# jacobkrantz/IVLN-CE

Hardware: AMD Instinct MI355X
Metric: env-steps/sec (batched MapCMA fwd+bwd) at 1/2/4/8 MI355X; t-nDTW parity (higher is better)
Workload: dtype f32

## Files before the change

ivln-ce_amd/build.py:

```python
import os
import subprocess
import sys

HERE = os.path.dirname(os.path.abspath(__file__))
CSRC = os.path.join(HERE, "csrc")
OUT = os.path.join(HERE, "libivln_hip.so")

SOURCES = {
    "mapper.hip": ["-ffp-contract=off"],
    "gemm_conv.hip": ["-mllvm", "-pragma-unroll-threshold=200000"],
    "conv_direct.hip": [],
    "gemm_vec.hip": ["-mllvm", "-pragma-unroll-threshold=200000"],
    "conv1x1_stream.hip": [],
    "conv_bf3.hip": [],
    "gn_conv.hip": [],
    "depth_net.hip": [],
    "cma_step.hip": [],
    "state_rnn.hip": [],
    "instr_rnn.hip": [],
    "nn_ops.hip": [],
    "train_ops.hip": [],
    "dtw.cpp": [],
}
COMMON = ["--offload-arch=gfx950", "-O3", "-std=c++17", "-fPIC", "-Wall", "-Wno-unused-function"]


def _stale(target, deps):
    if not os.path.exists(target):
        return True
    t = os.path.getmtime(target)
    return any(os.path.getmtime(d) > t for d in deps)


def build_all(force=False, verbose=True):
    hipcc = os.environ.get("HIPCC", "/opt/rocm/bin/hipcc")
    objs = []
    headers = [os.path.join(CSRC, f) for f in os.listdir(CSRC) if f.endswith((".h", ".hpp"))]
    headers.append(os.path.join(HERE, "..", "include", "ivln_hip.h"))
    procs = []
    for src, extra in SOURCES.items():
        s = os.path.join(CSRC, src)
        o = os.path.join(CSRC, src.rsplit(".", 1)[0] + ".o")
        objs.append(o)
        if force or _stale(o, [s] + headers):
            cmd = [hipcc] + COMMON + extra + ["-c", s, "-o", o]
            if verbose:
                print(" ".join(cmd), flush=True)
            procs.append((src, subprocess.Popen(cmd)))
    for src, p in procs:
        if p.wait() != 0:
            raise RuntimeError(f"hipcc failed on {src}")
    if force or procs or _stale(OUT, objs):
        cmd = [hipcc, "--offload-arch=gfx950", "-shared", "-fPIC", "-o", OUT] + objs
        if verbose:
            print(" ".join(cmd), flush=True)
        subprocess.check_call(cmd)
    return OUT


if __name__ == "__main__":
    build_all(force="--force" in sys.argv)
```

ivln-ce_amd/csrc/conv_bf3.hip:

```cpp
#include <stdlib.h>

#include <type_traits>

#include "bf3_common.h"
#include "residency.h"

namespace {

#ifdef BF3_TIMING
__device__ unsigned long long g_bf3_stamp[8192 * 8];
#endif

template <int KS, int TM, int WM, int WN, int PTH, int PTW, int IMGS, int DA, bool FUSE = false, int ST = 1>
__global__ __launch_bounds__(64 * WM * WN, 2) void k_conv_bf3(const ivln_gemm_desc p, const unsigned char* a_split, long long a_grp_bytes,
                                                           int tiles_w, int tiles_h, int nimg, int chunks_per_split) {
#ifdef BF3_TIMING
    const unsigned long long t_entry = threadIdx.x == 0 ? wall_clock64() : 0ull;
#endif
    constexpr int NTB = 64 * WM * WN, TN = 2;
    constexpr int BM = 32 * TM * WM, BN = 32 * TN * WN;
    static_assert(IMGS * PTH * PTW == BN && PTW % 4 == 0, "pixel tile");
    constexpr int KK = KS * KS, KKP = bf3_taps_padded(KS), CS = bf3_stage_chunks(KS);
    constexpr int RP = KKP * CS;
    static_assert(RP % DA == 0 && KKP >= KK && (CS == 1 || KK == 1), "prefetch rotation closes over a stage");
// ... 956 lines not shown
    float* const red = reinterpret_cast<float*>(smem);
    bf3_red_put<LDT>(red, wave, half, l31, acc);
    __syncthreads();
#pragma unroll
    for (int it = 0; it < ITEMS; ++it) {
        const int item = t + it * 512, ml = item >> 5, q = item & 31;
        float4 v = bf3_red_sum<NW, LDT, float4, 32>(red + ml * LDT + q);
        if (eoff[it] >= 0) {
            const int64_t addr = eoff[it];
            const float sc = esc[it], sh = esh[it];
            if (p.scale) v.x = fmaf(v.x, sc, sh), v.y = fmaf(v.y, sc, sh), v.z = fmaf(v.z, sc, sh), v.w = fmaf(v.w, sc, sh);
            else if (p.shift) v.x += sh, v.y += sh, v.z += sh, v.w += sh;
            const bool res_pre = p.residual && !p.residual_after_relu, res_post = p.residual && p.residual_after_relu;
            if (res_pre)
                v.x += __int_as_float(rres[it][0]), v.y += __int_as_float(rres[it][1]), v.z += __int_as_float(rres[it][2]),
                    v.w += __int_as_float(rres[it][3]);
            if (p.accumulate) {
                const float4 ra = *reinterpret_cast<const float4*>(p.D + addr);
                v.x += ra.x, v.y += ra.y, v.z += ra.z, v.w += ra.w;
            }
            if (p.relu) v.x = fmaxf(v.x, 0.f), v.y = fmaxf(v.y, 0.f), v.z = fmaxf(v.z, 0.f), v.w = fmaxf(v.w, 0.f);
            if (res_post)
                v.x += __int_as_float(rres[it][0]), v.y += __int_as_float(rres[it][1]), v.z += __int_as_float(rres[it][2]),
                    v.w += __int_as_float(rres[it][3]);
            *reinterpret_cast<float4*>(p.D + addr) = v;
        }
    }
    }
#ifdef BF3_TIMING
    if (lane == 0) {
        __builtin_amdgcn_s_waitcnt(0);
        const unsigned long long ts3 = wall_clock64();
        const int b = ((blockIdx.y * gridDim.x + blockIdx.x) * NW + wave) & 8191;
        g_bf3_stamp[b * 8 + 0] = ts1 - ts0;
        g_bf3_stamp[b * 8 + 1] = ts2 - ts1;
        g_bf3_stamp[b * 8 + 2] = ts3 - ts2;
        g_bf3_stamp[b * 8 + 3] = ts0;
        g_bf3_stamp[b * 8 + 4] = tc_split;
        g_bf3_stamp[b * 8 + 5] = tc_load;
        g_bf3_stamp[b * 8 + 6] = tc_mfma;
    }
#endif
}

int bf3_1x1_ks_launch(ivln_gemm_desc& d, hipStream_t s, int mode, int form_pin = -1) {
    if (d.stride != 1 || d.pad != 0 || d.Cin % CB != 0 || d.Cin < 4 * CB || d.stat_partials || d.splits > 1) return IVLN_E_UNSUPPORTED;
    if ((d.HoWo & 3) || (d.in_img_stride & 3) || ((((uintptr_t)d.B) | ((uintptr_t)d.D) | ((uintptr_t)d.residual)) & 15)) return IVLN_E_UNSUPPORTED;
    const int64_t nimg = d.N / d.HoWo;
    if (nimg * d.in_img_stride * 4 >= (int64_t)1 << 31 || nimg * d.Ctot * d.HoWo * 4 >= (int64_t)1 << 31) return IVLN_E_UNSUPPORTED;
    if (d.grp_imgs > 0 && ((int64_t)d.grp_imgs * d.HoWo) % 128 != 0) return IVLN_E_UNSUPPORTED;
    const int nch = d.Cin / CB;
    bool wt = nch <= 16;
    if (nch == 32 && (int64_t)((d.N + 127) / 128) * ((d.M + 31) / 32) > 2 * (int64_t)ivln_cu_count()) wt = true;
    if (form_pin >= 0) wt = form_pin == 1;
    if (wt && nch > 64) wt = false;
    if (wt && d.accumulate) return IVLN_E_UNSUPPORTED;
    const int64_t mtiles = (d.M + 31) / 32;
    const int64_t wgs = wt ? (int64_t)((d.N + 511) / 512) * mtiles : (int64_t)((d.N + 127) / 128) * mtiles;
    if ((d.N + 127) / 128 > 65535) return IVLN_E_UNSUPPORTED;
    if (mode == 0) {
        if (!wt && (d.Cin < 32 * CB || wgs > 2 * (int64_t)ivln_cu_count() || wgs < ivln_cu_count() / 2)) return IVLN_E_UNSUPPORTED;
        if (wt && wgs < ivln_cu_count()) return IVLN_E_UNSUPPORTED;
    }
    d.splits = 1;
    const unsigned char* a = (const unsigned char*)d.A_split;
    const long long gb = (long long)(d.a_split_grp_stride * 4);
    if (wt) {
        constexpr size_t lds = 0;
        dim3 grid((unsigned)mtiles, (unsigned)((d.N + 511) / 512), 1);
        IVLN_LAUNCH_FAMILY(k_conv1x1_bf3_ks<true>, grid, dim3(256), lds, s, d, a, gb);
    } else {
        constexpr size_t lds = (size_t)8 * 32 * (128 + 4) * 4;
        if (bf3_set_lds<k_conv1x1_bf3_ks<false>>(lds) != IVLN_OK) return IVLN_E_HIP;
        dim3 grid((unsigned)mtiles, (unsigned)((d.N + 127) / 128), 1);
        IVLN_LAUNCH_FAMILY(k_conv1x1_bf3_ks<false>, grid, dim3(512), lds, s, d, a, gb);
    }
    return IVLN_OK;
}

__global__ __launch_bounds__(256) void k_conv_bf3_pack(const float* __restrict__ W, int M, int Cin, int KS, uint16_t* __restrict__ out,
                                                       int64_t total) {
    const int64_t idx = (int64_t)blockIdx.x * 256 + threadIdx.x;
    if (idx >= total) return;
    const int KK = KS * KS, KKP = bf3_taps_padded(KS), nch = (Cin + CB - 1) / CB;
    const int e = (int)(idx & 7), lane = (int)((idx >> 3) & 63);
    int64_t q = idx >> 9;
    const int pl = (int)(q % 3);
    q /= 3;
    const int r = (int)(q % KKP);
    q /= KKP;
    const int c = (int)(q % nch);
    const int mt = (int)(q / nch);
    const int m = mt * 32 + (lane & 31), ci = c * CB + (lane >> 5) * 8 + e;
    const float v = (m < M && ci < Cin && r < KK) ? W[((int64_t)m * Cin + ci) * KK + r] : 0.f;
    uint32_t h, mm, l;
    split3(v, h, mm, l);
    out[idx] = (uint16_t)(pl == 0 ? h : (pl == 1 ? mm : l));
}

template <int KS, int TM, int WM, int WN, int PTH, int PTW, int IMGS, int DA, int ST = 1>
int launch_bf3(const ivln_gemm_desc& d, hipStream_t s, const unsigned char* a_split, int64_t grp_bytes, int nimg, int cps) {
    constexpr int NTB = 64 * WM * WN, BM = 32 * TM * WM, BN = 64 * WN;
    constexpr int PH = ST == 2 ? PTH + 1 : PTH + KS - 1, PWR = ST == 2 ? PTW + 1 : PTW + KS - 1;
    constexpr int NPIX = IMGS * (ST == 2 ? 4 : 1) * PH * PWR * bf3_stage_chunks(KS);
    constexpr size_t lds = (size_t)(NPIX * PIXB > 32 * (BN + 4) * 4 ? NPIX * PIXB : 32 * (BN + 4) * 4);
    if constexpr (lds > 160 * 1024) {
// ... 755 lines not shown
```

ivln-ce_amd/csrc/nn_ops.hip:

```cpp
#include <hip/hip_runtime.h>
#include <stdint.h>
#include <math.h>
#include "../../include/ivln_hip.h"

namespace {

__device__ __forceinline__ float wave_sum(float v) {
#pragma unroll
    for (int o = 32; o > 0; o >>= 1) v += __shfl_xor(v, o);
    return v;
}
__device__ __forceinline__ float wave_max(float v) {
#pragma unroll
    for (int o = 32; o > 0; o >>= 1) v = fmaxf(v, __shfl_xor(v, o));
    return v;
}
__device__ __forceinline__ float block_sum(float v, float* red) {
    v = wave_sum(v);
    int w = threadIdx.x >> 6, nw = (blockDim.x + 63) >> 6;
    __syncthreads();
    if ((threadIdx.x & 63) == 0) red[w] = v;
    __syncthreads();
    float s = 0.f;
    for (int i = 0; i < nw; ++i) s += red[i];
    return s;
}
__device__ __forceinline__ float block_max(float v, float* red) {
    v = wave_max(v);
    int w = threadIdx.x >> 6, nw = (blockDim.x + 63) >> 6;
    __syncthreads();
    if ((threadIdx.x & 63) == 0) red[w] = v;
    __syncthreads();
    float s = -INFINITY;
    for (int i = 0; i < nw; ++i) s = fmaxf(s, red[i]);
    return s;
}

constexpr int GN_CACHE = 8192;
constexpr int GN_THREADS = 512;

__device__ __forceinline__ float4 gn_load4(const float* __restrict__ xp, int i, int HW, int64_t chan_stride,
                                           int splits, int64_t slab_stride) {
    int cl = i / HW, pp = i - cl * HW;
    const float* p = xp + (int64_t)cl * chan_stride + pp;
    float4 v = *reinterpret_cast<const float4*>(p);
    int z = 1;
    for (; z + 3 < splits; z += 4) {
        float4 w0 = *reinterpret_cast<const float4*>(p + (int64_t)z * slab_stride);
        float4 w1 = *reinterpret_cast<const float4*>(p + (int64_t)(z + 1) * slab_stride);
        float4 w2 = *reinterpret_cast<const float4*>(p + (int64_t)(z + 2) * slab_stride);
        float4 w3 = *reinterpret_cast<const float4*>(p + (int64_t)(z + 3) * slab_stride);
        v.x += (w0.x + w1.x) + (w2.x + w3.x);
        v.y += (w0.y + w1.y) + (w2.y + w3.y);
        v.z += (w0.z + w1.z) + (w2.z + w3.z);
        v.w += (w0.w + w1.w) + (w2.w + w3.w);
    }
// ... 346 lines not shown
        float2 t2 = *reinterpret_cast<const float2*>(xp + (int64_t)z * slab_stride);
        float2 u2 = *reinterpret_cast<const float2*>(xp + (int64_t)z * slab_stride + W);
        t.x += t2.x; t.y += t2.y; u.x += u2.x; u.y += u2.y;
    }
    for (int off = lpo >> 1; off > 0; off >>= 1) {
        t.x += __shfl_xor(t.x, off, 64);
        t.y += __shfl_xor(t.y, off, 64);
        u.x += __shfl_xor(u.x, off, 64);
        u.y += __shfl_xor(u.y, off, 64);
    }
    if (!live || sub != 0) return;
    const float sc = scale[c], sh = shift[c];
    float a = fmaxf(fmaf(t.x, sc, sh), 0.f);
    float b = fmaxf(fmaf(t.y, sc, sh), 0.f);
    float c2 = fmaxf(fmaf(u.x, sc, sh), 0.f);
    float d = fmaxf(fmaf(u.y, sc, sh), 0.f);
    y[idx] = (((a + b) + c2) + d) * 0.25f;
}

__global__ __launch_bounds__(256) void k_pool2d(const float* __restrict__ x, float* __restrict__ y, int NC, int H,
                                                int W, int Ho, int Wo, int k, int s, int p, int mode) {
    int64_t idx = (int64_t)blockIdx.x * 256 + threadIdx.x;
    if (idx >= (int64_t)NC * Ho * Wo) return;
    int wo = (int)(idx % Wo);
    int ho = (int)((idx / Wo) % Ho);
    int nc = (int)(idx / ((int64_t)Wo * Ho));
    const float* xp = x + (int64_t)nc * H * W;
    float acc = mode == 0 ? -INFINITY : 0.f;
    for (int i = 0; i < k; ++i) {
        int h = ho * s - p + i;
        if ((unsigned)h >= (unsigned)H) continue;
        for (int j = 0; j < k; ++j) {
            int w = wo * s - p + j;
            if ((unsigned)w >= (unsigned)W) continue;
            float v = xp[(int64_t)h * W + w];
            acc = mode == 0 ? fmaxf(acc, v) : acc + v;
        }
    }
    if (mode == 1) acc = acc / (float)(k * k);
    y[idx] = acc;
}

__global__ __launch_bounds__(256) void k_subsample2_x4(const float* __restrict__ x, float* __restrict__ y, int64_t total4, int H, int W,
                                                      int Ho, int Wo) {
    const int64_t idx = (int64_t)blockIdx.x * 256 + threadIdx.x;
    if (idx >= total4) return;
    const int W4 = Wo >> 2;
    const int j = (int)(idx % W4);
    const int ho = (int)((idx / W4) % Ho);
    const int64_t nc = idx / ((int64_t)W4 * Ho);
    const float4* r = reinterpret_cast<const float4*>(x + (nc * H + 2 * ho) * W + 8 * j);
    const float4 a = r[0], b = r[1];
    *reinterpret_cast<float4*>(y + (nc * Ho + ho) * Wo + 4 * j) = make_float4(a.x, a.z, b.x, b.z);
}

__global__ __launch_bounds__(256) void k_maxpool3s2p1_x4(const float* __restrict__ x, float* __restrict__ y, int64_t total4, int H, int W,
                                                        int Ho, int Wo) {
    const int64_t idx = (int64_t)blockIdx.x * 256 + threadIdx.x;
    if (idx >= total4) return;
    const int W4 = Wo >> 2;
    const int j = (int)(idx % W4);
    const int ho = (int)((idx / W4) % Ho);
    const int64_t nc = idx / ((int64_t)W4 * Ho);
    const float* xp = x + nc * H * W;
    float m[9];
#pragma unroll
    for (int k = 0; k < 9; ++k) m[k] = -INFINITY;
#pragma unroll
    for (int i = 0; i < 3; ++i) {
        const int h = 2 * ho - 1 + i;
        if ((unsigned)h < (unsigned)H) {
            const float* r = xp + (int64_t)h * W + 8 * j;
            const float4 a = *reinterpret_cast<const float4*>(r), b = *reinterpret_cast<const float4*>(r + 4);
            const float l = j > 0 ? r[-1] : -INFINITY;
            m[0] = fmaxf(m[0], l), m[1] = fmaxf(m[1], a.x), m[2] = fmaxf(m[2], a.y), m[3] = fmaxf(m[3], a.z), m[4] = fmaxf(m[4], a.w);
            m[5] = fmaxf(m[5], b.x), m[6] = fmaxf(m[6], b.y), m[7] = fmaxf(m[7], b.z), m[8] = fmaxf(m[8], b.w);
        }
    }
    float4 o;
    o.x = fmaxf(fmaxf(m[0], m[1]), m[2]), o.y = fmaxf(fmaxf(m[2], m[3]), m[4]);
    o.z = fmaxf(fmaxf(m[4], m[5]), m[6]), o.w = fmaxf(fmaxf(m[6], m[7]), m[8]);
    *reinterpret_cast<float4*>(y + (nc * Ho + ho) * Wo + 4 * j) = o;
}

__global__ __launch_bounds__(256) void k_map_features(const uint8_t* __restrict__ occ,
                                                      const uint8_t* __restrict__ sem, float* __restrict__ y,
                                                      int B, int cells, int classes) {
    int64_t idx = (int64_t)blockIdx.x * 256 + threadIdx.x;
    int64_t total = (int64_t)B * (1 + classes) * cells;
    if (idx >= total) return;
    int p = (int)(idx % cells);
    int c = (int)((idx / cells) % (1 + classes));
    int b = (int)(idx / ((int64_t)cells * (1 + classes)));
    float v;
    if (c == 0) v = (float)occ[(int64_t)b * cells + p];
    else v = sem[(int64_t)b * cells + p] == (uint8_t)(c - 1) ? 1.f : 0.f;
    y[idx] = v;
}

__global__ __launch_bounds__(256) void k_map_features4(const uint8_t* __restrict__ occ, const uint8_t* __restrict__ sem,
                                                       float* __restrict__ y, int B, int cells, int classes) {
    const int64_t q = (int64_t)blockIdx.x * 256 + threadIdx.x;
    const int cq = cells >> 2;
    const int64_t total = (int64_t)B * (1 + classes) * cq;
    if (q >= total) return;
    const int p4 = (int)(q % cq);
// ... 881 lines not shown
                           const float* u_sample, const float* u_beta, float beta, const double* expert,
                           int64_t* action, float* logits_out, void* stream) {
    if (O > 8 || O <= 0 || (K & 3) || (ldx & 3) || rows <= 0) return IVLN_E_UNSUPPORTED;
    if (!u_sample || (u_beta && !expert)) return IVLN_E_INVALID;
    hipLaunchKernelGGL(k_linear_argmax<true>, dim3(1), dim3(256), 0, (hipStream_t)stream, x, ldx, W, bias, rows, K, O,
                       action, logits_out, u_sample, u_beta, beta, expert);
    return LAUNCH_OK();
}

int ivln_rgb_to_nchw_f32(const uint8_t* rgb, int B, int H, int W, float div, float* out, void* stream) {
    if (B <= 0 || div == 0.f) return IVLN_E_INVALID;
    hipLaunchKernelGGL(k_rgb_to_nchw, dim3(nblk((int64_t)B * H * W)), dim3(256), 0, (hipStream_t)stream, rgb, B, H, W,
                       div, out);
    return LAUNCH_OK();
}

int ivln_adaptive_avgpool2d_f32(const float* x, int N, int C, int H, int W, int OH, int OW, float* out,
                                int64_t out_img_stride, void* stream) {
    if (N <= 0 || OH <= 0 || OW <= 0) return IVLN_E_INVALID;
    if (out_img_stride <= 0) out_img_stride = (int64_t)C * OH * OW;
    hipLaunchKernelGGL(k_adaptive_avgpool2d, dim3(nblk((int64_t)N * C * OH * OW)), dim3(256), 0, (hipStream_t)stream, x,
                       N, C, H, W, OH, OW, out, out_img_stride);
    return LAUNCH_OK();
}

int ivln_argmax_channels_u8(const float* x, int N, int C, int HW, uint8_t* out, void* stream) {
    hipLaunchKernelGGL(k_argmax_channels_u8, dim3(nblk((int64_t)N * HW)), dim3(256), 0, (hipStream_t)stream, x, N, C,
                       HW, out);
    return LAUNCH_OK();
}

int ivln_rgb_resize_normalize_f32(const uint8_t* rgb, int B, int Hi, int Wi, int Ho, int Wo, float* out,
                                  void* stream) {
    if (Hi == Ho && Wi == Wo && ((int64_t)Ho * Wo) % 4 == 0 && !((uintptr_t)rgb & 3) && !((uintptr_t)out & 15)) {
        const int64_t quads = (int64_t)B * Ho * Wo / 4;
        hipLaunchKernelGGL(k_rgb_normalize_x4, dim3(nblk(quads)), dim3(256), 0, (hipStream_t)stream, rgb, quads, Ho * Wo, out);
        return LAUNCH_OK();
    }
    hipLaunchKernelGGL(k_rgb_resize_normalize, dim3(nblk((int64_t)B * 3 * Ho * Wo)), dim3(256), 0,
                       (hipStream_t)stream, rgb, B, Hi, Wi, Ho, Wo, out);
    return LAUNCH_OK();
}

int ivln_affine_f32(const float* x, float* y, int64_t n, float sub, float div, void* stream) {
    hipLaunchKernelGGL(k_affine, dim3(nblk(n)), dim3(256), 0, (hipStream_t)stream, x, y, n, sub, div);
    return LAUNCH_OK();
}

int ivln_add_f32(const float* a, const float* b, float* y, int64_t n, int relu, void* stream) {
    hipLaunchKernelGGL(k_add, dim3(nblk(n)), dim3(256), 0, (hipStream_t)stream, a, b, y, n, relu);
    return LAUNCH_OK();
}

int ivln_copy2d_f32(const float* src, int64_t ld_src, float* dst, int64_t ld_dst, int rows, int cols,
                    int broadcast_rows, void* stream) {
    hipLaunchKernelGGL(k_copy2d, dim3(nblk((int64_t)rows * cols)), dim3(256), 0, (hipStream_t)stream, src, ld_src,
                       dst, ld_dst, rows, cols, broadcast_rows);
    return LAUNCH_OK();
}

int ivln_copy_multi(const void* const* srcs, void* const* dsts, const int64_t* bytes, int n, void* stream) {
    if (n < 0 || n > 8) return IVLN_E_INVALID;
    CopyJobs J;
    int blocks = 0, m = 0;
    for (int j = 0; j < n; ++j) {
        if (bytes[j] <= 0) continue;
        if (!srcs[j] || !dsts[j]) return IVLN_E_INVALID;
        J.src[m] = (const uint8_t*)srcs[j];
        J.dst[m] = (uint8_t*)dsts[j];
        J.bytes[m] = bytes[j];
        J.first_block[m] = blocks;
        blocks += (int)((bytes[j] + COPY_CHUNK - 1) / COPY_CHUNK);
        ++m;
    }
    if (m == 0) return IVLN_OK;
    J.first_block[m] = blocks;
    J.n = m;
    hipLaunchKernelGGL(k_copy_multi, dim3(blocks), dim3(256), 0, (hipStream_t)stream, J);
    return LAUNCH_OK();
}

int ivln_rednet_fwd(const ivln_rednet_op* table, int n_ops, const uint8_t* rgb, const float* depth, uint8_t* labels_out,
                    void* stream) {
    if (!table || n_ops <= 0) return IVLN_E_INVALID;
    for (int k = 0; k < n_ops; ++k) {
        const ivln_rednet_op& op = table[k];
        int rc = IVLN_E_INVALID;
        switch (op.kind) {
            case IVLN_OP_GEMM:
                rc = ivln_gemm_f32(&op.gemm, stream);
                break;
            case IVLN_OP_ADD:
                rc = ivln_add_f32((const float*)op.src0, (const float*)op.src1, (float*)op.dst, op.n, op.i[0], stream);
                break;
            case IVLN_OP_POOL:
                rc = ivln_pool2d_f32((const float*)op.src0, (float*)op.dst, op.i[0], op.i[1], op.i[2], op.i[3], op.i[4],
                                     op.i[5], op.i[6], stream);
                break;
            case IVLN_OP_RGB_NORM: {
                const uint8_t* src = op.src0 ? (const uint8_t*)op.src0 : rgb;
                if (src)
                    rc = ivln_rgb_resize_normalize_f32(src, op.i[0], op.i[1], op.i[2], op.i[3], op.i[4], (float*)op.dst,
                                                       stream);
                break;
            }
            case IVLN_OP_AFFINE: {
                const float* src = op.src0 ? (const float*)op.src0 : depth;
                if (src) rc = ivln_affine_f32(src, (float*)op.dst, op.n, op.f[0], op.f[1], stream);
                break;
            }
            case IVLN_OP_ARGMAX_U8: {
                uint8_t* dst = op.dst ? (uint8_t*)op.dst : labels_out;
                if (dst) rc = ivln_argmax_channels_u8((const float*)op.src0, op.i[0], op.i[1], op.i[2], dst, stream);
                break;
            }
            default:
                break;
        }
        if (rc != IVLN_OK) return rc;
    }
    return IVLN_OK;
}

int ivln_add_multi_f32(const float* const* srcs, float* const* dsts, const int64_t* counts, int n, void* stream) {
    if (n < 0 || n > 64) return IVLN_E_INVALID;
    AddJobs J;
    int blocks = 0, m = 0;
    for (int j = 0; j < n; ++j) {
        if (counts[j] <= 0) continue;
        if (!srcs[j] || !dsts[j]) return IVLN_E_INVALID;
        J.src[m] = srcs[j];
        J.dst[m] = dsts[j];
        J.n[m] = counts[j];
        J.first_block[m] = blocks;
        blocks += (int)((counts[j] + ADD_CHUNK - 1) / ADD_CHUNK);
        ++m;
    }
    if (m == 0) return IVLN_OK;
    J.first_block[m] = blocks;
    J.count = m;
    hipLaunchKernelGGL(k_add_multi, dim3(blocks), dim3(256), 0, (hipStream_t)stream, J);
    return LAUNCH_OK();
}

}
```

ivln-ce_amd/ops.py:

```python
import ctypes as C
import contextlib
import functools
import os
from typing import Optional

import torch

from . import _lib
from ._lib import check, f32, i32, i64, lib, stream_ptr, vp
from ._lib import dptr as _dptr


class GemmDesc(C.Structure):

    _fields_ = [
        ("A", vp), ("B", vp), ("D", vp),
        ("M", i32), ("N", i32), ("K", i32),
        ("amode", i32), ("bmode", i32), ("dmode", i32),
        ("lda", i64), ("ldb", i64),
        ("Cin", i32), ("Hin", i32), ("Win", i32), ("Hout", i32), ("Wout", i32),
        ("stride", i32), ("pad", i32), ("dil", i32),
        ("koff", vp), ("kpos", vp),
        ("HoWo", i32), ("Ctot", i32),
        ("in_img_stride", i64),
        ("sDm", i64), ("sDn", i64),
        ("scale", vp), ("shift", vp), ("residual", vp),
        ("relu", i32), ("accumulate", i32),
        ("splits", i32),
        ("ws", vp), ("ws_floats", i64),
        ("defer_epilogue", i32), ("splits_used", C.POINTER(i32)),
        ("tile_override", i32),
        ("A_packed", vp),
        ("no_xcd_remap", i32),
        ("grp_imgs", i32), ("a_grp_stride", i64), ("a_packed_grp_stride", i64),
        ("no_wide_epilogue", i32),
        ("stat_partials", vp), ("stat_tiles", C.POINTER(i32)),
        ("A_split", vp), ("a_split_grp_stride", i64),
        ("split_ok", i32),
        ("img_run_flags", vp),
        ("fuse_A_split", vp), ("fuse_a_grp_stride", i64), ("fuse_scale", vp), ("fuse_shift", vp), ("fuse_M", i32),
        ("residual_after_relu", i32),
        ("real_taps", i32),
        ("pool2", i32), ("map_sem_u8", vp),
    ]


class RednetOp(C.Structure):
    _fields_ = [("kind", i32), ("i", i32 * 7), ("f", f32 * 2), ("n", i64), ("src0", vp), ("src1", vp), ("dst", vp),
                ("gemm", GemmDesc)]


OP_GEMM, OP_ADD, OP_POOL, OP_RGB_NORM, OP_AFFINE, OP_ARGMAX_U8 = range(6)


class OpRecorder:

    def __init__(self):
        self.ops, self.keep, self.unsupported = [], [], []

    def table(self):
        arr = (RednetOp * len(self.ops))()
        for k, op in enumerate(self.ops):
            C.memmove(C.byref(arr, k * C.sizeof(RednetOp)), C.byref(op), C.sizeof(RednetOp))
        return arr


_REC = None


class recording:
    def __enter__(self):
        global _REC
        if _REC is not None:
            raise _lib.IvlnError("ops.recording() does not nest")
        _REC = OpRecorder()
        return _REC

    def __exit__(self, *exc):
        global _REC
        _REC = None
        return False


def _rec(kind, ints=(), floats=(), n=0, src0=None, src1=None, dst=None, gemm=None):
    op = RednetOp()
    op.kind = kind
    for k, v in enumerate(ints):
        op.i[k] = int(v)
    for k, v in enumerate(floats):
        op.f[k] = float(v)
    op.n, op.src0, op.src1, op.dst = int(n), src0, src1, dst
    if gemm is not None:
        C.memmove(C.byref(op, RednetOp.gemm.offset), C.byref(gemm), C.sizeof(GemmDesc))
        op.gemm.splits_used = None
    _REC.ops.append(op)


A_MK, A_KM, A_NCHW_P = 0, 1, 2
B_CONV, B_CONV1X1, B_KN, B_NK, B_IM2COL_T, B_CONVT, B_CONV_K3, B_CONV_K7, B_CONV_K2 = 0, 1, 2, 3, 4, 5, 6, 7, 8
D_NCHW, D_DENSE, D_NCHW_UP2, D_NCHW_UP2X4 = 0, 1, 2, 3

_sigs_done = False


def _L():
    global _sigs_done
    L = lib()
    if not _sigs_done:
        L.ivln_gemm_f32.argtypes = [C.POINTER(GemmDesc), vp]
        L.ivln_groupnorm_f32.argtypes = [vp, vp, vp, vp, vp, i32, i32, i32, i32, f32, i32, i64, i64, i32, i64, i64, i64,
                                         vp, vp, vp]
        L.ivln_bn_fold_f32.argtypes = [vp, vp, vp, vp, vp, f32, i32, vp, vp, vp]
        L.ivln_bn_train_stats_f32.argtypes = [vp, i32, i32, i32, vp, vp, vp, vp, f32, f32, vp, vp, vp, vp, vp, i64, vp]
        L.ivln_scale_shift_relu_avgpool2_f32.argtypes = [vp, vp, vp, vp, i32, i32, i32, i32, i64, i64, i32, i64, vp]
        L.ivln_pool2d_f32.argtypes = [vp, vp, i32, i32, i32, i32, i32, i32, i32, vp]
        L.ivln_map_features_f32.argtypes = [vp, vp, vp, i32, i32, i32, vp]
        L.ivln_embed_lengths.argtypes = [vp, vp, i32, i32, i32, i32, vp, vp, vp]
        L.ivln_embed_gates_dirs_f32.argtypes = [vp, vp, vp, i32, i32, i32, i32, i32, vp, vp, vp, vp, vp, vp]
        L.ivln_lstm_dirs_fwd_f32.argtypes = [vp] * 7 + [i32, i32, i32, i32, vp, vp, vp, vp, i32, vp, vp]
        L.ivln_gru_dirs_fwd_f32.argtypes = [vp] * 7 + [i32, i32, i32, i32, vp, vp, vp, vp]
        L.ivln_linear_skinny_f32.argtypes = [vp, i64, vp, vp, vp, i64, i32, i32, i32, i32, vp]
        L.ivln_gru_step_f32.argtypes = [vp, i64, i32, vp, i64, vp, i64, vp, vp, vp, vp, vp, vp, i64, vp, i64, i32, i32,
                                        vp, vp, vp, vp, vp]
        L.ivln_attn_fwd_f32.argtypes = [vp, i64, vp, i64, vp, i64, vp, f32, i32, i32, i32, i32, vp, i64, vp, vp, vp]
        L.ivln_prev_action_embed_f32.argtypes = [vp, vp, vp, i32, i32, i32, vp, i64, vp, i64, vp]
        L.ivln_argmax_rows.argtypes = [vp, i32, i32, vp, vp]
        L.ivln_argmax_channels_u8.argtypes = [vp, i32, i32, i32, vp, vp]
        L.ivln_rgb_resize_normalize_f32.argtypes = [vp, i32, i32, i32, i32, i32, vp, vp]
        L.ivln_affine_f32.argtypes = [vp, vp, i64, f32, f32, vp]
        L.ivln_add_f32.argtypes = [vp, vp, vp, i64, i32, vp]
        L.ivln_copy2d_f32.argtypes = [vp, i64, vp, i64, i32, i32, i32, vp]
        L.ivln_tour_memory_f32.argtypes = [vp, i64, vp, i64, vp, i32, i32, vp, i64, vp, i64, vp]
        L.ivln_seq_sync_init.argtypes = L.ivln_seq_sync_status.argtypes = [vp, vp]
        L.ivln_cma_seq_fwd_f32.argtypes = [vp, vp, i64, vp, vp, vp, vp, i64, vp, i64, i32, i32, i32, vp, vp, vp, vp, vp, vp]
        L.ivln_lstm_step_f32.argtypes = [vp, i64, i32, vp, i64, vp, i64, vp, i64, vp, vp, vp, vp, vp, vp, i64, vp, i64, vp,
                                         i64, i32, i32, vp, vp, vp, vp, vp, vp]
        L.ivln_lstm_seq_fwd_f32.argtypes = [vp, vp, i64, vp, i64, vp, vp, vp, vp, i64, vp, i64, vp, i64, i32, i32, i32, vp,
                                            vp, vp, vp, vp, vp]
        L.ivln_lstm_seq_bwd_f32.argtypes = [vp, i64, vp, vp, vp, vp, vp, vp, i64, vp, i64, vp, i64, vp, vp, i32, i32, i32,
                                            vp, vp, vp, i64, vp, i64, vp]
        _sigs_done = True
    return L


def dptr(t: torch.Tensor) -> int:
    if _REC is not None:
        _REC.keep.append(t)
    return _dptr(t)


def _p(t: Optional[torch.Tensor]):
    if t is None:
        return None
    if not t.is_cuda:
        raise _lib.IvlnError("HIP hot path needs GPU tensors (no CPU fallback); got " + str(t.device))
    if _REC is not None:
        _REC.keep.append(t)
    return t.data_ptr()


_tables = {}
_ws = {}


def conv_tables(cin, kh, kw, hin, win, dil, device, transposed=False):
    key = (cin, kh, kw, hin, win, dil, str(device), transposed)
    t = _tables.get(key)
    if t is None:
        ci = torch.arange(cin, dtype=torch.int64).view(-1, 1, 1)
        a = torch.arange(kh, dtype=torch.int64).view(1, -1, 1)
        b = torch.arange(kw, dtype=torch.int64).view(1, 1, -1)
        if transposed:
            koff = (ci * hin * win + 0 * a + 0 * b).reshape(-1)
        else:
            koff = (ci * hin * win + a * dil * win + b * dil).reshape(-1)
        kpos = (0 * ci + (a << 16) + b).reshape(-1)
        t = (koff.to(torch.int32).to(device), kpos.to(torch.int32).to(device))
        _tables[key] = t
    return t


def splitk_ws(device, floats=8 << 20, slot=0):
    key = (str(device), stream_ptr(), slot)
# ... 1189 lines not shown
    check(_L().ivln_argmax_channels_u8(dptr(x), N, Cc, H * W, dptr(out), stream_ptr()), "ivln_argmax_channels_u8")
    if _REC is not None:
        _rec(OP_ARGMAX_U8, (N, Cc, H * W), src0=x.data_ptr(), dst=None)
    return out


def rgb_resize_normalize(rgb_u8_nhwc, Ho, Wo):
    B, Hi, Wi, _ = rgb_u8_nhwc.shape
    out = torch.empty((B, 3, Ho, Wo), dtype=torch.float32, device=rgb_u8_nhwc.device)
    check(_L().ivln_rgb_resize_normalize_f32(dptr(rgb_u8_nhwc), B, Hi, Wi, Ho, Wo, dptr(out), stream_ptr()),
          "ivln_rgb_resize_normalize_f32")
    if _REC is not None:
        _rec(OP_RGB_NORM, (B, Hi, Wi, Ho, Wo), src0=None, dst=out.data_ptr())
    return out


def rgb_to_nchw(rgb_u8_nhwc, div=255.0):
    B, H, W, _ = rgb_u8_nhwc.shape
    out = torch.empty((B, 3, H, W), dtype=torch.float32, device=rgb_u8_nhwc.device)
    L = _L()
    L.ivln_rgb_to_nchw_f32.argtypes = [vp, i32, i32, i32, f32, vp, vp]
    check(L.ivln_rgb_to_nchw_f32(dptr(rgb_u8_nhwc), B, H, W, div, dptr(out), stream_ptr()), "ivln_rgb_to_nchw_f32")
    return out


def adaptive_avgpool2d(x, OH, OW, out=None, out_ctot=0):
    N, Cc, H, W = x.shape
    if out is None:
        out = torch.empty((N, Cc, OH, OW), dtype=torch.float32, device=x.device)
    L = _L()
    L.ivln_adaptive_avgpool2d_f32.argtypes = [vp, i32, i32, i32, i32, i32, i32, vp, i64, vp]
    check(L.ivln_adaptive_avgpool2d_f32(dptr(x), N, Cc, H, W, OH, OW, _p(out), out_ctot * OH * OW, stream_ptr()),
          "ivln_adaptive_avgpool2d_f32")
    return out


def affine(x, sub, div):
    out = torch.empty_like(x)
    check(_L().ivln_affine_f32(dptr(x), dptr(out), x.numel(), sub, div, stream_ptr()), "ivln_affine_f32")
    if _REC is not None:
        _rec(OP_AFFINE, floats=(sub, div), n=x.numel(), src0=None, dst=out.data_ptr())
    return out


def add(a, b, relu=False, out=None):
    if out is None:
        out = torch.empty_like(a)
    check(_L().ivln_add_f32(dptr(a), dptr(b), dptr(out), a.numel(), int(bool(relu)), stream_ptr()), "ivln_add_f32")
    if _REC is not None:
        _rec(OP_ADD, (int(bool(relu)),), n=a.numel(), src0=a.data_ptr(), src1=b.data_ptr(), dst=out.data_ptr())
    return out


def copy_multi(pairs):
    L = _L()
    L.ivln_copy_multi.argtypes = [C.POINTER(C.c_void_p), C.POINTER(C.c_void_p), C.POINTER(C.c_int64), C.c_int,
                                  C.c_void_p]
    for k in range(0, len(pairs), 8):
        chunk = pairs[k:k + 8]
        n = len(chunk)
        srcs, dsts, nb = (C.c_void_p * n)(), (C.c_void_p * n)(), (C.c_int64 * n)()
        for i, (s, d) in enumerate(chunk):
            if s.shape != d.shape or s.dtype != d.dtype or not s.is_contiguous() or not d.is_contiguous():
                raise _lib.IvlnError("copy_multi needs contiguous tensors of identical shape and dtype")
            srcs[i], dsts[i], nb[i] = _p(s), _p(d), s.numel() * s.element_size()
        check(L.ivln_copy_multi(srcs, dsts, nb, n, stream_ptr()), "ivln_copy_multi")


def add_multi(pairs):
    L = _L()
    L.ivln_add_multi_f32.argtypes = [C.POINTER(C.c_void_p), C.POINTER(C.c_void_p), C.POINTER(C.c_int64), C.c_int,
                                     C.c_void_p]
    for k in range(0, len(pairs), 64):
        chunk = pairs[k:k + 64]
        n = len(chunk)
        srcs, dsts, cnt = (C.c_void_p * n)(), (C.c_void_p * n)(), (C.c_int64 * n)()
        for i, (s, d) in enumerate(chunk):
            if (s.numel() != d.numel() or s.dtype != torch.float32 or d.dtype != torch.float32
                    or not s.is_contiguous() or not d.is_contiguous()):
                raise _lib.IvlnError("add_multi needs contiguous float32 tensors of identical size")
            srcs[i], dsts[i], cnt[i] = _p(s), _p(d), s.numel()
        check(L.ivln_add_multi_f32(srcs, dsts, cnt, n, stream_ptr()), "ivln_add_multi_f32")


def tour_memory(mem, h, mask_u8, out1, out2=None):
    N, H = mem.shape
    check(
        _L().ivln_tour_memory_f32(_p(mem), mem.stride(0), _p(h) if h is not None else None, h.stride(0) if h is not None else 0,
                                  _p(mask_u8) if mask_u8 is not None else None, N, H, _p(out1), out1.stride(0),
                                  _p(out2) if out2 is not None else None, out2.stride(0) if out2 is not None else 0,
                                  stream_ptr()),
        "ivln_tour_memory_f32",
    )
    return out1


def copy2d(src, dst, rows, cols, broadcast_rows=False):
    check(
        _L().ivln_copy2d_f32(_p(src), src.stride(0) if src.dim() > 1 else cols, _p(dst), dst.stride(0), rows, cols,
                             int(bool(broadcast_rows)), stream_ptr()),
        "ivln_copy2d_f32",
    )


_tsigs_done = False

# ... 375 lines not shown
```

ivln-ce_amd/rednet.py:

```python
import os

import torch
import torch.nn as nn

from . import ops


GROUP_ENCODERS = True


def _conv3x3(cin, cout, stride=1):
    return nn.Conv2d(cin, cout, kernel_size=3, stride=stride, padding=1, bias=False)


class _Folded:

    def __init__(self):
        self.c = {}

    def bn(self, bn: nn.BatchNorm2d):
        k = id(bn)
        if k not in self.c:
            C = bn.num_features
            scale = torch.empty(C, dtype=torch.float32, device=bn.weight.device)
            shift = torch.empty(C, dtype=torch.float32, device=bn.weight.device)
            ops.bn_fold(bn, scale, shift)
            self.c[k] = (scale, shift)
        return self.c[k]

    def pair(self, conv_a, bn_a, conv_b, bn_b):
        k = ("pair", id(conv_a))
        if k not in self.c:
            (sa, ba), (sb, bb) = self.bn(bn_a), self.bn(bn_b)
            w = torch.stack([conv_a.weight.detach(), conv_b.weight.detach()]).contiguous()
            self.c[k] = (w, torch.cat([sa, sb]).contiguous(), torch.cat([ba, bb]).contiguous())
        return self.c[k]

    def classes(self, convt: nn.ConvTranspose2d):
        k = ("cls", id(convt))
        if k not in self.c:
            ok = convt.stride == (2, 2) and convt.kernel_size[0] == convt.kernel_size[1] and \
                2 - 2 * convt.padding[0] + convt.kernel_size[0] - 2 + convt.output_padding[0] == 2
            cls = ops.convt_s2_classes(convt.weight.detach(), convt.padding[0]) if ok else None
            self.c[k] = None if cls is None else (cls, ops.convt_s2_stack(cls))
        return self.c[k]

    def wt(self, convt: nn.ConvTranspose2d):
        k = id(convt)
        if k not in self.c:
            self.c[k] = convt.weight.detach().permute(1, 0, 2, 3).contiguous()
        return self.c[k]


def _convt(x, convt: nn.ConvTranspose2d, f: _Folded, **epi):
    cls = f.classes(convt)
    if cls is not None:
        return ops.conv_transpose2d_s2(x, cls[0], stacked=cls[1], **epi)
    return ops.conv_transpose2d(x, f.wt(convt), convt.stride[0], convt.padding[0], convt.output_padding[0], **epi)


STAGE_HOOK = None


def _stage_done(name):
    if STAGE_HOOK is not None:
        STAGE_HOOK(name)


SKIP_ADD_FUSED = os.environ.get("IVLN_REDNET_SKIP_ADD", "1") != "0"


class Bottleneck(nn.Module):
    expansion = 4

    def __init__(self, inplanes, planes, stride=1, downsample=None):
        super().__init__()
        self.conv1 = nn.Conv2d(inplanes, planes, kernel_size=1, bias=False)
        self.bn1 = nn.BatchNorm2d(planes)
        self.conv2 = nn.Conv2d(planes, planes, kernel_size=3, stride=stride, padding=1, bias=False)
        self.bn2 = nn.BatchNorm2d(planes)
        self.conv3 = nn.Conv2d(planes, planes * 4, kernel_size=1, bias=False)
        self.bn3 = nn.BatchNorm2d(planes * 4)
        self.relu = nn.ReLU(inplace=True)
        self.downsample = downsample
        self.stride = stride

    def forward_hip(self, x, f: _Folded):
        residual = x
        if self.downsample is not None:
            s, b = f.bn(self.downsample[1])
            residual = ops.conv2d(x, self.downsample[0].weight, stride=self.stride, scale=s, shift=b)
        s, b = f.bn(self.bn1)
        y = ops.conv2d(x, self.conv1.weight, scale=s, shift=b, relu=True)
        s, b = f.bn(self.bn2)
        s3, b3 = f.bn(self.bn3)
        if self.stride == 1:
            out = ops.conv3x3_then_1x1(y, self.conv2.weight, s, b, self.conv3.weight, s3, b3, residual)
            if out is not None:
                return out
        y = ops.conv2d(y, self.conv2.weight, stride=self.stride, pad=1, scale=s, shift=b, relu=True)
        return ops.conv2d(y, self.conv3.weight, scale=s3, shift=b3, residual=residual, relu=True)


def _conv_pair(x2, w2, s2, b2, stride=1, pad=0, residual=None, relu=False):
    N, _, H, W = x2.shape
    G, Cout, _, KH, KW = w2.shape
    B = N // G
    Ho, Wo = (H + 2 * pad - KH) // stride + 1, (W + 2 * pad - KW) // stride + 1
    if (B * Ho * Wo) % 32 == 0:
        return ops.conv2d(x2, w2, stride=stride, pad=pad, scale=s2, shift=b2, residual=residual, relu=relu)
    out = torch.empty((N, Cout, Ho, Wo), dtype=torch.float32, device=x2.device)
    for g in range(G):
        sl = slice(g * B, (g + 1) * B)
        ops.conv2d(x2[sl], w2[g], stride=stride, pad=pad, scale=s2[g * Cout:(g + 1) * Cout], shift=b2[g * Cout:(g + 1) * Cout],
                   residual=residual[sl] if residual is not None else None, relu=relu, out=out[sl])
    return out


def _bottleneck_pair(blk: Bottleneck, blk_d: Bottleneck, x2, f: _Folded):
    residual = x2
    if blk.downsample is not None:
        w, s, b = f.pair(blk.downsample[0], blk.downsample[1], blk_d.downsample[0], blk_d.downsample[1])
        residual = _conv_pair(x2, w, s, b, stride=blk.stride)
    w, s, b = f.pair(blk.conv1, blk.bn1, blk_d.conv1, blk_d.bn1)
    y = _conv_pair(x2, w, s, b, relu=True)
    w, s, b = f.pair(blk.conv2, blk.bn2, blk_d.conv2, blk_d.bn2)
    w3, s3, b3 = f.pair(blk.conv3, blk.bn3, blk_d.conv3, blk_d.bn3)
    if blk.stride == 1:
        out = ops.conv3x3_then_1x1(y, w, s, b, w3, s3, b3, residual)
        if out is not None:
            return out
    y = _conv_pair(y, w, s, b, stride=blk.stride, pad=1, relu=True)
    return _conv_pair(y, w3, s3, b3, residual=residual, relu=True)


class TransBasicBlock(nn.Module):
    expansion = 1

    def __init__(self, inplanes, planes, stride=1, upsample=None, **kwargs):
        super().__init__()
        self.conv1 = _conv3x3(inplanes, inplanes)
        self.bn1 = nn.BatchNorm2d(inplanes)
        self.relu = nn.ReLU(inplace=True)
        if upsample is not None and stride != 1:
            self.conv2 = nn.ConvTranspose2d(inplanes, planes, kernel_size=3, stride=stride, padding=1,
                                            output_padding=1, bias=False)
        else:
            self.conv2 = _conv3x3(inplanes, planes, stride)
        self.bn2 = nn.BatchNorm2d(planes)
        self.upsample = upsample
        self.stride = stride

    def forward_hip(self, x, f: _Folded):
        residual = x
        if self.upsample is not None:
            s, b = f.bn(self.upsample[1])
            up = self.upsample[0]
            if isinstance(up, nn.ConvTranspose2d):
                residual = _convt(x, up, f, scale=s, shift=b)
            else:
                residual = ops.conv2d(x, up.weight, scale=s, shift=b)
        s, b = f.bn(self.bn1)
        y = ops.conv2d(x, self.conv1.weight, pad=1, scale=s, shift=b, relu=True)
        s, b = f.bn(self.bn2)
        if isinstance(self.conv2, nn.ConvTranspose2d):
            return _convt(y, self.conv2, f, scale=s, shift=b, residual=residual, relu=True)
        return ops.conv2d(y, self.conv2.weight, stride=self.stride, pad=1, scale=s, shift=b, residual=residual,
                          relu=True)


class RedNet(nn.Module):
    def __init__(self, cfg):
# ... 55 lines not shown
            upsample = nn.Sequential(
                nn.ConvTranspose2d(self.inplanes, planes, kernel_size=2, stride=stride, padding=0, bias=False),
                nn.BatchNorm2d(planes),
            )
        elif self.inplanes != planes:
            upsample = nn.Sequential(
                nn.Conv2d(self.inplanes, planes, kernel_size=1, stride=stride, bias=False), nn.BatchNorm2d(planes)
            )
        layers = [block(self.inplanes, self.inplanes) for _ in range(1, blocks)]
        layers.append(block(self.inplanes, planes, stride, upsample))
        self.inplanes = planes
        return nn.Sequential(*layers)

    def _make_agant_layer(self, inplanes, planes):
        return nn.Sequential(
            nn.Conv2d(inplanes, planes, kernel_size=1, stride=1, padding=0, bias=False),
            nn.BatchNorm2d(planes), nn.ReLU(inplace=True),
        )

    def invalidate_folded(self):
        self._folded = _Folded()

    def _seq(self, seq, x):
        for blk in seq:
            x = blk.forward_hip(x, self._folded)
        return x

    def _agant(self, layer, x):
        s, b = self._folded.bn(layer[1])
        return ops.conv2d(x, layer[0].weight, scale=s, shift=b, relu=True)

    def _skip_add(self, up, layer, fuse):
        s, b = self._folded.bn(layer[1])
        out = ops.conv2d(fuse, layer[0].weight, scale=s, shift=b, residual=up, relu=True, residual_after_relu=True) if SKIP_ADD_FUSED else None
        return out if out is not None else ops.add(up, self._agant(layer, fuse))

    def forward(self, rgb, depth):
        assert not self.training, "HIP RedNet is inference-only (the reference freezes it, mapper.py:751-752)"
        f = self._folded
        if GROUP_ENCODERS:
            B = rgb.shape[0]
            S = torch.empty((2 * B, 64, rgb.shape[2] // 2, rgb.shape[3] // 2), dtype=torch.float32, device=rgb.device)
            s, b = f.bn(self.bn1)
            sd, bd = f.bn(self.bn1_d)
            ops.conv2d(depth, self.conv1_d.weight, stride=2, pad=3, scale=sd, shift=bd, relu=True, out=S[B:])
            fuse0 = ops.conv2d(rgb, self.conv1.weight, stride=2, pad=3, scale=s, shift=b, relu=True, out=S[:B], residual=S[B:],
                               residual_after_relu=True) if ops.BF3_STEM else None
            if fuse0 is None:
                ops.conv2d(rgb, self.conv1.weight, stride=2, pad=3, scale=s, shift=b, relu=True, out=S[:B])
                fuse0 = ops.add(S[:B], S[B:], out=S[:B])
            P = ops.pool2d(S, 3, 2, 1, "max")
            fuses = []
            _stage_done("stem")
            for li, (la, lb) in enumerate(((self.layer1, self.layer1_d), (self.layer2, self.layer2_d),
                                           (self.layer3, self.layer3_d), (self.layer4, self.layer4_d))):
                for blk, blk_d in zip(la, lb):
                    P = _bottleneck_pair(blk, blk_d, P, f)
                fuses.append(ops.add(P[:B], P[B:], out=P[:B]))
                _stage_done(f"layer{li + 1}")
            fuse1, fuse2, fuse3, fuse4 = fuses
        else:
            s, b = f.bn(self.bn1)
            x = ops.conv2d(rgb, self.conv1.weight, stride=2, pad=3, scale=s, shift=b, relu=True)
            s, b = f.bn(self.bn1_d)
            d = ops.conv2d(depth, self.conv1_d.weight, stride=2, pad=3, scale=s, shift=b, relu=True)
            fuse0 = ops.add(x, d)
            x = ops.pool2d(fuse0, 3, 2, 1, "max")
            d = ops.pool2d(d, 3, 2, 1, "max")
            x, d = self._seq(self.layer1, x), self._seq(self.layer1_d, d)
            fuse1 = ops.add(x, d)
            x, d = self._seq(self.layer2, fuse1), self._seq(self.layer2_d, d)
            fuse2 = ops.add(x, d)
            x, d = self._seq(self.layer3, fuse2), self._seq(self.layer3_d, d)
            fuse3 = ops.add(x, d)
            x, d = self._seq(self.layer4, fuse3), self._seq(self.layer4_d, d)
            fuse4 = ops.add(x, d)
        x = self._agant(self.agant4, fuse4)
        for di, (seq, ag, fuse) in enumerate(((self.deconv1, self.agant3, fuse3), (self.deconv2, self.agant2, fuse2),
                                              (self.deconv3, self.agant1, fuse1), (self.deconv4, self.agant0, fuse0))):
            x = self._skip_add(self._seq(seq, x), ag, fuse)
            _stage_done(f"deconv{di + 1}")
        x = self._seq(self.final_conv, x)
        fd = self.final_deconv_custom
        return _convt(x, fd, f, shift=fd.bias)


class PredictSemantics:

    CFG = {
        "arch": "rednet", "resnet_pretrained": False, "finetune": True, "SUNRGBD_pretrained_weights": "",
        "n_classes": 13, "upsample_prediction": True, "load_model": "data/rednet_mp3d_best_model.pkl",
    }

    def __init__(self, device, model: RedNet = None, load_weights: bool = True):
        self.device = device
        self.model = model
        self.load_weights = load_weights

    def setup(self):
        if self.model is None:
            self.model = RedNet(self.CFG)
            path = self.CFG["load_model"]
            if self.load_weights and os.path.exists(path):
                state = torch.load(path, map_location="cpu")["model_state"]
                if next(iter(state)).split(".")[0] == "module":
                    state = {".".join(k.split(".")[1:]): v for k, v in state.items()}
                self.model.load_state_dict(state)
            self.model = self.model.to(self.device).eval()
            for p in self.model.parameters():
                p.requires_grad = False

# ... 40 lines not shown
```

Baseline: 2448.

## Merge downsample into conv3 for stride-2 entry blocks and fuse add with subsample gather

```diff
diff --git a/include/ivln_rednet_glue.h b/include/ivln_rednet_glue.h
--- /dev/null
+++ b/include/ivln_rednet_glue.h
@@ -0,0 +1,15 @@
+#ifndef IVLN_REDNET_GLUE_H
+#define IVLN_REDNET_GLUE_H
+#include "ivln_hip.h"
+#ifdef __cplusplus
+extern "C" {
+#endif
+
+int ivln_add_subsample2_f32(float* x, int B, int C, int H, int W, int add, float* dst, int dst_ctot, int dst_coff, void* stream);
+
+enum { IVLN_OP_ADD_SUBSAMPLE2 = 6 };
+
+#ifdef __cplusplus
+}
+#endif
+#endif
diff --git a/ivln-ce_amd/build.py b/ivln-ce_amd/build.py
--- a/ivln-ce_amd/build.py
+++ b/ivln-ce_amd/build.py
@@ -37,6 +37,7 @@
     objs = []
     headers = [os.path.join(CSRC, f) for f in os.listdir(CSRC) if f.endswith((".h", ".hpp"))]
     headers.append(os.path.join(HERE, "..", "include", "ivln_hip.h"))
+    headers.append(os.path.join(HERE, "..", "include", "ivln_rednet_glue.h"))
     procs = []
     for src, extra in SOURCES.items():
         s = os.path.join(CSRC, src)
diff --git a/ivln-ce_amd/csrc/conv_bf3.hip b/ivln-ce_amd/csrc/conv_bf3.hip
--- a/ivln-ce_amd/csrc/conv_bf3.hip
+++ b/ivln-ce_amd/csrc/conv_bf3.hip
@@ -1032,6 +1032,7 @@
     const int nch = d.Cin / CB;
     bool wt = nch <= 16;
     if (nch == 32 && (int64_t)((d.N + 127) / 128) * ((d.M + 31) / 32) > 2 * (int64_t)ivln_cu_count()) wt = true;
+    if ((nch == 24 || nch == 48) && (int64_t)((d.N + 127) / 128) * ((d.M + 31) / 32) > 2 * (int64_t)ivln_cu_count()) wt = true;
     if (form_pin >= 0) wt = form_pin == 1;
     if (wt && nch > 64) wt = false;
     if (wt && d.accumulate) return IVLN_E_UNSUPPORTED;
diff --git a/ivln-ce_amd/csrc/nn_ops.hip b/ivln-ce_amd/csrc/nn_ops.hip
--- a/ivln-ce_amd/csrc/nn_ops.hip
+++ b/ivln-ce_amd/csrc/nn_ops.hip
@@ -2,6 +2,7 @@
 #include <stdint.h>
 #include <math.h>
 #include "../../include/ivln_hip.h"
+#include "../../include/ivln_rednet_glue.h"
 
 namespace {
 
@@ -454,6 +455,33 @@
     const float4* r = reinterpret_cast<const float4*>(x + (nc * H + 2 * ho) * W + 8 * j);
     const float4 a = r[0], b = r[1];
     *reinterpret_cast<float4*>(y + (nc * Ho + ho) * Wo + 4 * j) = make_float4(a.x, a.z, b.x, b.z);
+}
+
+template <bool ADD>
+__global__ __launch_bounds__(256) void k_add_subsample2_x4(float* __restrict__ x, float* __restrict__ dst, int64_t total8, int B, int C,
+                                                          int H, int W, int ctot, int coff) {
+    const int64_t idx = (int64_t)blockIdx.x * 256 + threadIdx.x;
+    if (idx >= total8) return;
+    const int W8 = W >> 3, Ho = H >> 1, Wo = W >> 1;
+    const int j = (int)(idx % W8);
+    const int h = (int)((idx / W8) % H);
+    if (!ADD && (h & 1)) return;
+    const int64_t nc = idx / ((int64_t)W8 * H);
+    float4* const pa = reinterpret_cast<float4*>(x + (nc * H + h) * W + 8 * j);
+    float4 a0 = pa[0], a1 = pa[1];
+    float4 b0 = make_float4(0.f, 0.f, 0.f, 0.f), b1 = b0;
+    if (ADD) {
+        const float4* const pb = reinterpret_cast<const float4*>(x + (int64_t)B * C * H * W + (nc * H + h) * W + 8 * j);
+        b0 = pb[0], b1 = pb[1];
+        a0.x += b0.x, a0.y += b0.y, a0.z += b0.z, a0.w += b0.w;
+        a1.x += b1.x, a1.y += b1.y, a1.z += b1.z, a1.w += b1.w;
+        pa[0] = a0, pa[1] = a1;
+        if (h & 1) return;
+    }
+    const int n = (int)(nc / C), c = (int)(nc - (int64_t)n * C);
+    const int64_t o = (((int64_t)n * ctot + coff + c) * Ho + (h >> 1)) * Wo + 4 * j;
+    *reinterpret_cast<float4*>(dst + o) = make_float4(a0.x, a0.z, a1.x, a1.z);
+    if (ADD) *reinterpret_cast<float4*>(dst + o + (int64_t)B * ctot * Ho * Wo) = make_float4(b0.x, b0.z, b1.x, b1.z);
 }
 
 __global__ __launch_bounds__(256) void k_maxpool3s2p1_x4(const float* __restrict__ x, float* __restrict__ y, int64_t total4, int H, int W,
@@ -1441,6 +1469,20 @@
     return LAUNCH_OK();
 }
 
+int ivln_add_subsample2_f32(float* x, int B, int C, int H, int W, int add, float* dst, int dst_ctot, int dst_coff, void* stream) {
+    if (!x || !dst || B <= 0 || C <= 0 || H <= 0 || W <= 0 || (H & 1) || (W & 7) || dst_coff < 0 || dst_coff + C > dst_ctot ||
+        ((((uintptr_t)x) | ((uintptr_t)dst)) & 15))
+        return IVLN_E_INVALID;
+    const int64_t total8 = (int64_t)B * C * H * (W / 8);
+    if (add)
+        hipLaunchKernelGGL(k_add_subsample2_x4<true>, dim3(nblk(total8)), dim3(256), 0, (hipStream_t)stream, x, dst, total8, B, C, H, W,
+                           dst_ctot, dst_coff);
+    else
+        hipLaunchKernelGGL(k_add_subsample2_x4<false>, dim3(nblk(total8)), dim3(256), 0, (hipStream_t)stream, x, dst, total8, B, C, H, W,
+                           dst_ctot, dst_coff);
+    return LAUNCH_OK();
+}
+
 int ivln_copy2d_f32(const float* src, int64_t ld_src, float* dst, int64_t ld_dst, int rows, int cols,
                     int broadcast_rows, void* stream) {
     hipLaunchKernelGGL(k_copy2d, dim3(nblk((int64_t)rows * cols)), dim3(256), 0, (hipStream_t)stream, src, ld_src,
@@ -1503,6 +1545,10 @@
                 if (dst) rc = ivln_argmax_channels_u8((const float*)op.src0, op.i[0], op.i[1], op.i[2], dst, stream);
                 break;
             }
+            case IVLN_OP_ADD_SUBSAMPLE2:
+                rc = ivln_add_subsample2_f32((float*)op.src0, op.i[0], op.i[1], op.i[2], op.i[3], op.i[6], (float*)op.dst, op.i[4], op.i[5],
+                                             stream);
+                break;
             default:
                 break;
         }
diff --git a/ivln-ce_amd/ops.py b/ivln-ce_amd/ops.py
--- a/ivln-ce_amd/ops.py
+++ b/ivln-ce_amd/ops.py
@@ -50,7 +50,7 @@
                 ("gemm", GemmDesc)]
 
 
-OP_GEMM, OP_ADD, OP_POOL, OP_RGB_NORM, OP_AFFINE, OP_ARGMAX_U8 = range(6)
+OP_GEMM, OP_ADD, OP_POOL, OP_RGB_NORM, OP_AFFINE, OP_ARGMAX_U8, OP_ADD_SUBSAMPLE2 = range(7)
 
 
 class OpRecorder:
@@ -129,6 +129,7 @@
         L.ivln_rgb_resize_normalize_f32.argtypes = [vp, i32, i32, i32, i32, i32, vp, vp]
         L.ivln_affine_f32.argtypes = [vp, vp, i64, f32, f32, vp]
         L.ivln_add_f32.argtypes = [vp, vp, vp, i64, i32, vp]
+        L.ivln_add_subsample2_f32.argtypes = [vp, i32, i32, i32, i32, i32, vp, i32, i32, vp]
         L.ivln_copy2d_f32.argtypes = [vp, i64, vp, i64, i32, i32, i32, vp]
         L.ivln_tour_memory_f32.argtypes = [vp, i64, vp, i64, vp, i32, i32, vp, i64, vp, i64, vp]
         L.ivln_seq_sync_init.argtypes = L.ivln_seq_sync_status.argtypes = [vp, vp]
@@ -1424,6 +1425,17 @@
     return out
 
 
+def add_subsample2(x, B, dst, coff=0, add=True):
+    N, Cc, H, W = x.shape
+    if N != (2 * B if add else B) or tuple(dst.shape) != (N, dst.shape[1], H // 2, W // 2) or H % 2 or W % 8:
+        raise _lib.IvlnError(f"add_subsample2: x {tuple(x.shape)}, dst {tuple(dst.shape)}, B {B}")
+    check(_L().ivln_add_subsample2_f32(dptr(x), B, Cc, H, W, int(bool(add)), dptr(dst), dst.shape[1], coff, stream_ptr()),
+          "ivln_add_subsample2_f32")
+    if _REC is not None:
+        _rec(OP_ADD_SUBSAMPLE2, (B, Cc, H, W, dst.shape[1], coff, int(bool(add))), src0=x.data_ptr(), dst=dst.data_ptr())
+    return x[:B] if add else x
+
+
 def copy_multi(pairs):
     L = _L()
     L.ivln_copy_multi.argtypes = [C.POINTER(C.c_void_p), C.POINTER(C.c_void_p), C.POINTER(C.c_int64), C.c_int,
diff --git a/ivln-ce_amd/rednet.py b/ivln-ce_amd/rednet.py
--- a/ivln-ce_amd/rednet.py
+++ b/ivln-ce_amd/rednet.py
@@ -7,6 +7,8 @@
 
 
 GROUP_ENCODERS = True
+MERGE_ENTRY_CONV3 = True
+FUSE_ADD_GATHER = True
 
 
 def _conv3x3(cin, cout, stride=1):
@@ -34,6 +36,21 @@
             (sa, ba), (sb, bb) = self.bn(bn_a), self.bn(bn_b)
             w = torch.stack([conv_a.weight.detach(), conv_b.weight.detach()]).contiguous()
             self.c[k] = (w, torch.cat([sa, sb]).contiguous(), torch.cat([ba, bb]).contiguous())
+        return self.c[k]
+
+    def merged3(self, blk, blk_d=None):
+        k = ("m3", id(blk.conv3), blk_d is not None)
+        if k not in self.c:
+            def one(b):
+                (sd, bd), (s3, b3) = self.bn(b.downsample[1]), self.bn(b.bn3)
+                wd, w3 = b.downsample[0].weight.detach(), b.conv3.weight.detach()
+                return torch.cat([wd * sd.view(-1, 1, 1, 1), w3 * s3.view(-1, 1, 1, 1)], dim=1), b3 + bd
+            if blk_d is None:
+                w, sh = one(blk)
+                self.c[k] = (w.contiguous(), sh)
+            else:
+                (wa, sa), (wb, sb) = one(blk), one(blk_d)
+                self.c[k] = (torch.stack([wa, wb]).contiguous(), torch.cat([sa, sb]).contiguous())
         return self.c[k]
 
     def classes(self, convt: nn.ConvTranspose2d):
@@ -86,6 +103,10 @@
         self.stride = stride
 
     def forward_hip(self, x, f: _Folded):
+        if _entry_merge_ok(self, x, 1):
+            buf = _entry_buf(self, x)
+            ops.add_subsample2(x, x.shape[0], buf, add=False)
+            return _entry_merged(self, None, x, buf, f)
         residual = x
         if self.downsample is not None:
             s, b = f.bn(self.downsample[1])
@@ -117,7 +138,37 @@
     return out
 
 
-def _bottleneck_pair(blk: Bottleneck, blk_d: Bottleneck, x2, f: _Folded):
+def _entry_merge_ok(blk: Bottleneck, x, G):
+    if not MERGE_ENTRY_CONV3 or not ops.S2_GATHER or blk.stride != 2 or blk.downsample is None or not x.is_contiguous():
+        return False
+    N, _, H, W = x.shape
+    return H % 2 == 0 and W % 8 == 0 and (G == 1 or (N % G == 0 and (N // G * (H // 2) * (W // 2)) % 128 == 0))
+
+
+def _entry_buf(blk: Bottleneck, x):
+    N, Cin, H, W = x.shape
+    return torch.empty((N, Cin + blk.conv2.out_channels, H // 2, W // 2), dtype=torch.float32, device=x.device)
+
+
+def _entry_merged(blk: Bottleneck, blk_d, x, buf, f: _Folded):
+    Cin, Ctot = x.shape[1], buf.shape[1]
+    if blk_d is None:
+        w1, (s1, b1), w2, (s2, b2) = blk.conv1.weight, f.bn(blk.bn1), blk.conv2.weight, f.bn(blk.bn2)
+    else:
+        w1, s1, b1 = f.pair(blk.conv1, blk.bn1, blk_d.conv1, blk_d.bn1)
+        w2, s2, b2 = f.pair(blk.conv2, blk.bn2, blk_d.conv2, blk_d.bn2)
+    y = ops.conv2d(x, w1, scale=s1, shift=b1, relu=True)
+    ops.conv2d(y, w2, stride=2, pad=1, scale=s2, shift=b2, relu=True, out=buf[:, Cin:], out_ctot=Ctot)
+    wm, shm = f.merged3(blk, blk_d)
+    return ops.conv2d(buf, wm, shift=shm, relu=True)
+
+
+def _bottleneck_pair(blk: Bottleneck, blk_d: Bottleneck, x2, f: _Folded, entry_buf=None):
+    if entry_buf is not None or _entry_merge_ok(blk, x2, 2):
+        if entry_buf is None:
+            entry_buf = _entry_buf(blk, x2)
+            ops.add_subsample2(x2, x2.shape[0], entry_buf, add=False)
+        return _entry_merged(blk, blk_d, x2, entry_buf, f)
     residual = x2
     if blk.downsample is not None:
         w, s, b = f.pair(blk.downsample[0], blk.downsample[1], blk_d.downsample[0], blk_d.downsample[1])
@@ -279,11 +330,19 @@
             P = ops.pool2d(S, 3, 2, 1, "max")
             fuses = []
             _stage_done("stem")
-            for li, (la, lb) in enumerate(((self.layer1, self.layer1_d), (self.layer2, self.layer2_d),
-                                           (self.layer3, self.layer3_d), (self.layer4, self.layer4_d))):
-                for blk, blk_d in zip(la, lb):
-                    P = _bottleneck_pair(blk, blk_d, P, f)
-                fuses.append(ops.add(P[:B], P[B:], out=P[:B]))
+            layers = ((self.layer1, self.layer1_d), (self.layer2, self.layer2_d), (self.layer3, self.layer3_d),
+                      (self.layer4, self.layer4_d))
+            buf = None
+            for li, (la, lb) in enumerate(layers):
+                for bi, (blk, blk_d) in enumerate(zip(la, lb)):
+                    P = _bottleneck_pair(blk, blk_d, P, f, entry_buf=buf if bi == 0 else None)
+                nxt = layers[li + 1][0][0] if li + 1 < len(layers) else None
+                if FUSE_ADD_GATHER and nxt is not None and _entry_merge_ok(nxt, P, 2):
+                    buf = _entry_buf(nxt, P)
+                    fuses.append(ops.add_subsample2(P, B, buf))
+                else:
+                    buf = None
+                    fuses.append(ops.add(P[:B], P[B:], out=P[:B]))
                 _stage_done(f"layer{li + 1}")
             fuse1, fuse2, fuse3, fuse4 = fuses
         else:
```

After: 2491, median of 6. 1.02x the previous value.
